# ZhengyiLuo/PHC

Measured on AMD Instinct MI355X. Metric: env-steps/sec at 4096 humanoid envs per GPU (VecEnv.step incl. resets), higher is better.
Workload: dtype f32

## Files before the change

### phc_amd/csrc/phc_im.h

```cpp
#pragma once
#include "phc_task.h"

namespace phc {

#if defined(PHC_SIM_PROFILE) && defined(__HIPCC__)
static __device__ unsigned long long g_phc_ptl[32];
static __device__ long long g_phc_ptl_env = -1;
#if defined(__HIP_DEVICE_COMPILE__)
#define PHC_PTL(i, ENV, LANE) if ((long long)(ENV) == g_phc_ptl_env) { __builtin_amdgcn_sched_barrier(0); __builtin_amdgcn_s_waitcnt(0); \
        const unsigned long long t_ = __builtin_readcyclecounter(); if ((LANE) == 0) g_phc_ptl[i] = t_; __builtin_amdgcn_sched_barrier(0); }
#else
#define PHC_PTL(i, ENV, LANE)
#endif
#else
#define PHC_PTL(i, ENV, LANE)
#endif

PHC_HD int64_t motion_id_of(const phc_im_buffers_t& buf, int64_t env) { return buf.sampled_motion_ids ? buf.sampled_motion_ids[env] : env; }

PHC_HD int phc_atomic_inc(int32_t* p) {
#if defined(__HIP_DEVICE_COMPILE__)
    return atomicAdd(p, 1);
#else
    int v;
#pragma omp atomic capture
    v = (*p)++;
    return v;
#endif
}

PHC_HD void amp_obs_from_frames_lane(const phc_motion_lib_t& lib, const phc_im_params_t& prm, int nb, int j, const FrameRef& fr, float* a);
PHC_HD void amp_obs_from_ref_lane(const phc_motion_lib_t& lib, const phc_im_params_t& prm, int nb, int j,
                                  int64_t mid, float t, float* a) {
    if (j < nb && prm.num_amp_obs_extra > 0 && prm.amp_obs_extra)
        obs_extra_lane(prm.amp_obs_extra + mid * prm.num_amp_obs_extra, prm.num_amp_obs_extra, j, nb, a + prm.num_amp_obs_per_step - prm.num_amp_obs_extra);
    amp_obs_from_frames_lane(lib, prm, nb, j, frame_ref(lib, mid, t), a);
}
PHC_HD void amp_obs_from_frames_lane(const phc_motion_lib_t& lib, const phc_im_params_t& prm, int nb, int j, const FrameRef& fr, float* a) {
    BodyState root = ref_body(lib, fr, 0);
    Q4 hinv = calc_heading_quat_inv(obs_root_rot(prm, root.rot));
    if (j == 0) amp_obs_root(prm, root.pos, root.rot, root.vel, root.angvel, hinv, a);
    if (j >= 1 && j < nb) {
        int slot = prm.amp_joint_slot[j];
        if (slot >= 0) {
            V3 dp, dv;
            if (prm.dofs_per_joint == 1) {
                ref_joint(lib, fr, j, &dp, &dv);
                amp_obs_joint(prm, slot, dp, dv, a);
            } else {
                Q4 lr;
                ref_joint_rot(lib, fr, j, &lr, &dv);
                amp_obs_joint_rot(prm, slot, lr, dv, a);
            }
        }
    }
    if (j < prm.num_key_bodies) {
        BodyState kb = ref_body(lib, fr, prm.key_body_ids[j]);
        amp_obs_key(prm, j, kb.pos, kb.vel, root.pos, hinv, a);
    }
}

PHC_HD void amp_obs_from_sim_lane(const phc_im_params_t& prm, const phc_sim_state_t& sim, int nb, int nd, int64_t env, int j,
                                  const BodyState& root, Q4 hinv, const int* dof_start_tab, float* a) {
    if (j < nb && prm.num_amp_obs_extra > 0 && prm.amp_obs_extra)
        obs_extra_lane(prm.amp_obs_extra + env * prm.num_amp_obs_extra, prm.num_amp_obs_extra, j, nb, a + prm.num_amp_obs_per_step - prm.num_amp_obs_extra);
    if (j == 0) amp_obs_root(prm, root.pos, root.rot, root.vel, root.angvel, hinv, a);
    if (j >= 1 && j < nb) {
        int slot = prm.amp_joint_slot[j];
        if (slot >= 0) {
            V3 dp, dv;
            ld_joint_state(sim, nd, env, dof_start_tab[j], prm.dofs_per_joint, &dp, &dv);
            amp_obs_joint(prm, slot, dp, dv, a);
        }
    }
    if (j < prm.num_key_bodies) {
        BodyState kb = load_body(sim.rigid_body_state, env, nb, prm.key_body_ids[j]);
        amp_obs_key(prm, j, kb.pos, kb.vel, root.pos, hinv, a);
    }
}

PHC_HD int64_t amp_env_stride(const phc_im_params_t& prm, const phc_im_buffers_t& buf) {
    return buf.amp_env_stride > 0 ? buf.amp_env_stride : (int64_t)prm.num_amp_obs_steps * prm.num_amp_obs_per_step;
}
PHC_HD void amp_shift_lane(const phc_im_params_t& prm, const phc_im_buffers_t& buf, int64_t env, int lane, int nl) {
    const int A = prm.num_amp_obs_per_step, S = prm.num_amp_obs_steps;
    if (buf.amp_obs_out + A == buf.amp_obs_in) return;
    const float* src = buf.amp_obs_in + env * amp_env_stride(prm, buf);
    float* dst = buf.amp_obs_out + env * amp_env_stride(prm, buf) + A;
    const int n = (S - 1) * A;
    if ((A & 3) == 0) {
        const float4* s4 = reinterpret_cast<const float4*>(src);
        float4* d4 = reinterpret_cast<float4*>(dst);
        int i = lane;
        for (; i + 3 * nl < n / 4; i += 4 * nl) {
            const float4 a = s4[i], b = s4[i + nl], c = s4[i + 2 * nl], e = s4[i + 3 * nl];
            d4[i] = a; d4[i + nl] = b; d4[i + 2 * nl] = c; d4[i + 3 * nl] = e;
        }
        for (; i < n / 4; i += nl) d4[i] = s4[i];
    } else {
        for (int i = lane; i < n; i += nl) dst[i] = src[i];
    }
}

struct ImStepCtx {
    int64_t progress;
    float t_rew; V3 goff_rew;
    float t0; V3 goff;
    float t1;
    float start, start_off;
    int pass_time;
    int cycled, cycle_cnt, recovery_cnt;
};

PHC_HD ImStepCtx im_post_prologue(const phc_motion_lib_t& lib, const phc_im_params_t& prm, const phc_sim_state_t& sim,
                                  const phc_im_buffers_t& buf, int64_t env, int64_t progress) {
    ImStepCtx c;
    const int64_t mid = motion_id_of(buf, env);
    c.start = buf.motion_start_times[env];
    c.start_off = buf.motion_start_times_offset[env];
    c.goff_rew = ld3(buf.global_offset + env * 3);
    c.goff = c.goff_rew;
    c.t_rew = motion_time(progress, prm.dt, c.start, c.start_off);
    c.t0 = c.t_rew;
    c.cycle_cnt = buf.cycle_counter ? (buf.cycle_counter[env] > 1 ? buf.cycle_counter[env] - 1 : 0) : 0;
    c.recovery_cnt = buf.recovery_counter ? (buf.recovery_counter[env] > 1 ? buf.recovery_counter[env] - 1 : 0) : 0;
    c.cycled = 0;
    const bool pass_len = c.t_rew >= lib.motion_lengths[mid];
    c.pass_time = pass_len ? 1 : 0;
    if (prm.cycle_motion) {
        c.pass_time = (progress >= (int64_t)prm.max_episode_length - 1) ? 1 : 0;
        if (pass_len) {
            c.cycled = 1;
            c.start_off = neg_progress_time(progress, prm.dt);
            c.start = sample_time_interval(lib, mid, buf.cycle_phase[env]);
            c.cycle_cnt = 60;
            const FrameRef fr = frame_ref(lib, mid, c.start);
            const V3 rp = ref_root_pos_lerp(lib, fr);
            const float* rs = sim.root_states + env * 13;
            c.goff.x = rs[0] - rp.x; c.goff.y = rs[1] - rp.y;
            if (buf.offset_rand && prm.cycle_motion_xp) {
                c.goff.x += buf.offset_rand[env * 2]; c.goff.y += buf.offset_rand[env * 2 + 1];
            } else if (buf.offset_rand && prm.zero_out_far && prm.zero_out_far_train) {
                float ox, oy;
                disk_offset(buf.offset_rand[env * 2], buf.offset_rand[env * 2 + 1], &ox, &oy);
                c.goff.x += ox; c.goff.y += oy;
            }
            c.t0 = motion_time(progress, prm.dt, c.start, c.start_off);
        }
    }
    c.progress = progress;
    if (c.recovery_cnt > 0) c.progress = progress - 1;
    c.t1 = motion_time(c.progress + 1, prm.dt, c.start, c.start_off);
    return c;
}

PHC_HD float zero_out_far_ref(const phc_im_params_t& prm, int slot, const BodyState& body, const BodyState& root,
                              const BodyState& ref_root, BodyState* ref) {
    const float distance = norm(root.pos - ref_root.pos);
    if (distance > prm.close_distance) {
        if (slot >= 1) { ref->pos = body.pos; ref->rot = body.rot; }
        ref->vel = body.vel; ref->angvel = body.angvel;
    }
    if (distance > prm.far_distance && slot == 0) {
        V3 d = ref->pos - body.pos;
        ref->pos = v3(d.x / distance * prm.far_distance, d.y / distance * prm.far_distance, d.z / distance * prm.far_distance) + body.pos;
    }
    return distance;
}

PHC_HD bool occluded(const phc_im_buffers_t& buf, const phc_im_params_t& prm, int64_t env, int slot) {
    return buf.occl_mask != nullptr && slot >= 0 && buf.occl_mask[env * prm.num_track_bodies + slot] != 0;
}
PHC_HD void occlude_ref(const phc_im_buffers_t& buf, const phc_im_params_t& prm, int64_t env, int slot, const BodyState& body, BodyState* rt) {
    if (!occluded(buf, prm, env, slot) || (prm.obs_v >= 1 && prm.obs_v <= 3)) return;
    if (prm.obs_v == 7) { rt->pos = body.pos; rt->rot = body.rot; }
    else *rt = body;
}

PHC_HD void task_obs_future_lane(const phc_motion_lib_t& lib, const phc_im_params_t& prm, int64_t mid, int64_t progress1, float start, float start_off,
                                 V3 goff, int slot, int j, const BodyState& body, const BodyState& root, float* tobs) {
    const int T = prm.num_traj_samples;
    if (T <= 1 || slot < 0 || !(prm.obs_v == 6 || prm.obs_v == 7 || prm.obs_v == 9)) return;
    const Q4 hroot = obs_root_rot(prm, root.rot);
    const Q4 hinv = calc_heading_quat_inv(hroot), h = calc_heading_quat(hroot);
    const int block = prm.num_task_obs / T;
    for (int k = 1; k < T; ++k) {
        PHC_NO_CONTRACT
        const float kts = (float)k * prm.traj_sample_timestep;
        BodyState r = ref_body(lib, frame_ref(lib, mid, motion_time_future(progress1, prm.dt, kts, start, start_off)), j);
        r.pos += goff;
        task_obs_lane(prm, slot, body, root, r, hinv, h, tobs + k * block);
    }
}

PHC_HD RewardPartial im_post_lane(const phc_model_t& model, const phc_motion_lib_t& lib, const phc_im_params_t& prm,
                                  const phc_sim_state_t& sim, const phc_im_buffers_t& buf, int64_t env, int j, const ImStepCtx& c,
                                  const FrameTab& tab, const BodyState& body, const BodyState& root) {
    const int nb = model.num_bodies, nd = model.num_dof;
    RewardPartial rp;
    rp.pos = rp.rot = rp.vel = rp.angvel = rp.power = rp.dist = rp.root_dist = 0.f; rp.fallen = 0;
    const int64_t mid = motion_id_of(buf, env);
    if (j >= nb) {
        const int e = j - nb;
        if (e >= prm.num_ext_bodies || prm.track_body_reward) return rp;
        const BodyState par = load_body(sim.rigid_body_state, env, nb, prm.ext_parent[e]);
        BodyState cur;
        cur.pos = quat_rotate(par.rot, ld3(prm.ext_offset + 3 * e)) + par.pos;
        cur.rot = par.rot;
        BodyState ref;
        ref_body_ext(lib, frame_ref(lib, mid, c.cycled ? c.t_rew : c.t0), e, &ref.pos, &ref.rot);
        ref.pos += c.cycled ? c.goff_rew : c.goff;
        const V3 d = ref.pos - cur.pos;
        rp.pos = (d.x * d.x + d.y * d.y + d.z * d.z) / 3.0f;
        const float ang = quat_to_angle_axis(quat_mul(ref.rot, quat_conjugate(cur.rot)), nullptr);
        rp.rot = ang * ang;
        return rp;
    }
    const FrameRef fr0 = frame_ref(tab, c.t0), fr1 = frame_ref(tab, c.t1);
    PHC_PTL(2, env, j)
    const BodyRaw q0 = ref_body_raw(lib, fr0, j), q1 = ref_body_raw(lib, fr1, j);
    JointPosRaw qj;
    const bool want_dof = buf.ref_dof_pos != nullptr && j >= 1;
    if (want_dof) qj = ref_joint_pos_raw(lib, fr1, j);
    PHC_PTL(3, env, j)
    const Q4 hroot = obs_root_rot(prm, root.rot);
    Q4 hinv = calc_heading_quat_inv(hroot), h = calc_heading_quat(hroot);
    float* obs = buf.obs_buf + env * (int64_t)(prm.num_self_obs + prm.num_task_obs);
    if (prm.self_obs_v == 2 && buf.body_state_hist) self_obs_v2_lane(prm, buf.body_state_hist, nb, env, j, body, root, hinv, obs, true, false);
    else self_obs_lane(prm, nb, j, body, root, hinv, obs, (sim.force_sensor && prm.self_obs_v == 3) ? sim.force_sensor + env * (int64_t)(prm.num_force_sensors * 6) : nullptr, env);
    PHC_PTL(4, env, j)
    {
        float* amp = buf.amp_obs_out + env * amp_env_stride(prm, buf);
        amp_obs_from_sim_lane(prm, sim, nb, nd, env, j, root, hinv, model.ints + 4 + 3 * PHC_MAX_BODIES, amp);
    }
    PHC_PTL(5, env, j)
    BodyState r0 = ref_body_blend(q0, fr0.blend), r1 = ref_body_blend(q1, fr1.blend);
    r0.pos += c.goff; r1.pos += c.goff;
    rp = reward_partial(prm, env, nb, j, body, r0);
    if (c.cycled) {
        BodyState rr = ref_body(lib, frame_ref(lib, mid, c.t_rew), j);
        rr.pos += c.goff_rew;
        RewardPartial q = reward_partial(prm, env, nb, j, body, rr);
        rp.pos = q.pos; rp.rot = q.rot; rp.vel = q.vel; rp.angvel = q.angvel;
        if (j == 0) rp.root_dist = norm(body.pos - rr.pos);
    } else if (j == 0) {
        rp.root_dist = norm(body.pos - r0.pos);
    }
    if (prm.track_body_reward && prm.track_slot[j] < 0) rp.pos = rp.rot = rp.vel = rp.angvel = 0.f;
    if (occluded(buf, prm, env, prm.track_slot[j])) { rp.dist = 0.f; rp.fallen = 0; }
    if (prm.power_reward && j >= 1) {
        int ds = model.ints[4 + 3 * PHC_MAX_BODIES + j];
        const float* d = sim.dof_state + (env * nd + ds) * 2;
        const float* f = sim.dof_force + env * nd + ds;
        rp.power = fabsf(f[0] * d[1]);
        if (prm.dofs_per_joint != 1) rp.power += fabsf(f[1] * d[3]) + fabsf(f[2] * d[5]);
    }
    PHC_PTL(6, env, j)
    int slot = prm.track_slot[j];
    if (slot >= 0) {
        BodyState rt = r1;
        if (prm.zero_out_far && !(prm.obs_v >= 1 && prm.obs_v <= 3)) {
            BodyState rroot = (j == 0) ? r1 : ref_body(lib, fr1, 0);
            if (j != 0) rroot.pos += c.goff;
            const float dist = zero_out_far_ref(prm, slot, body, root, rroot, &rt);
            if (j == 0 && buf.point_goal) buf.point_goal[env] = dist;
        }
        occlude_ref(buf, prm, env, slot, body, &rt);
        V3 jd = v3(0.f, 0.f, 0.f), jv, rjd = jd, rjv;
        if (prm.obs_v == 2 && j >= 1) {
            ld_joint_state(sim, nd, env, model.ints[4 + 3 * PHC_MAX_BODIES + j], prm.dofs_per_joint, &jd, &jv);
            ref_joint(lib, fr1, j, &rjd, &rjv);
        }
        task_obs_lane(prm, slot, body, root, rt, hinv, h, obs + prm.num_self_obs, &jd, &rjd);
    }
    PHC_PTL(7, env, j)
    if (buf.ref_body_pos) st3(buf.ref_body_pos + (env * nb + j) * 3, r1.pos);
    if (buf.ref_body_rot) st4(buf.ref_body_rot + (env * nb + j) * 4, r1.rot);
    if (buf.ref_body_vel) st3(buf.ref_body_vel + (env * nb + j) * 3, r1.vel);
    if (want_dof)
        st_joint(buf.ref_dof_pos + env * nd + model.ints[4 + 3 * PHC_MAX_BODIES + j], prm.dofs_per_joint, ref_joint_pos_blend(lib, qj, fr1.blend));
    PHC_PTL(8, env, j)
    if (prm.num_traj_samples > 1)
        task_obs_future_lane(lib, prm, mid, c.progress + 1, c.start, c.start_off, c.goff, prm.track_slot[j], j, load_body(sim.rigid_body_state, env, nb, j),
                             load_body(sim.rigid_body_state, env, nb, 0), buf.obs_buf + env * (int64_t)(prm.num_self_obs + prm.num_task_obs) + prm.num_self_obs);
    return rp;
}

PHC_HD void im_post_finalize(const phc_motion_lib_t& lib, const phc_im_params_t& prm, const phc_im_buffers_t& buf, int nb,
                             int64_t env, const ImStepCtx& c, int64_t progress, float s_pos, float s_rot, float s_vel, float s_angvel,
                             float s_power, float s_dist, float root_dist, float prev_point_goal, int any_fallen, int n_reset_bodies) {
    float J = (float)nb, JE = (float)(nb + prm.num_ext_bodies);
    if (prm.track_body_reward) J = JE = (float)prm.num_track_bodies;
    float r_pos = expf(-prm.k_pos * (s_pos / JE));
    float r_rot = expf(-prm.k_rot * (s_rot / JE));
    float r_vel = expf(-prm.k_vel * (s_vel / J));
    float r_ang = expf(-prm.k_ang_vel * (s_angvel / J));
    float rew = prm.w_pos * r_pos + prm.w_rot * r_rot + prm.w_vel * r_vel + prm.w_ang_vel * r_ang;
    const int nraw = prm.power_reward ? 5 : 4;
    float* raw = buf.reward_raw + env * nraw;
    if (prm.zero_out_far) {
        const float pg = fminf(prev_point_goal - root_dist, 1.0f / 3.0f) * 9.0f;
        const bool far = root_dist > 0.25f;
        raw[0] = pg + (far ? 0.f : r_pos * 0.5f);
        raw[1] = far ? 0.f : r_rot * 0.5f; raw[2] = far ? 0.f : r_vel * 0.5f; raw[3] = far ? 0.f : r_ang * 0.5f;
        rew = pg + (far ? 0.f : rew * 0.5f);
    } else {
        raw[0] = r_pos; raw[1] = r_rot; raw[2] = r_vel; raw[3] = r_ang;
    }
    if (prm.power_reward) {
        float pr = -prm.power_coefficient * s_power;
        if (progress <= 3) pr = 0.f;
        rew += pr;
        raw[4] = pr;
    }
    buf.rew_buf[env] = rew;
    int fallen = any_fallen;
    if (prm.use_mean_termination) {
        float mean = s_dist / (float)n_reset_bodies;
        fallen = mean > prm.termination_distances[prm.first_reset_body] ? 1 : 0;
    }
    int64_t terminated = 0;
    if (prm.enable_early_termination) {
        if (!(progress > 1)) fallen = 0;
        if (prm.disable_collision_check) fallen = 0;
        terminated = fallen ? 1 : 0;
    }
    int64_t reset = c.pass_time ? 1 : terminated;
    if (!c.pass_time && c.cycle_cnt > 0) { reset = 0; terminated = 0; }
    if (c.recovery_cnt > 0) { reset = 0; terminated = 0; }
    buf.terminate_buf[env] = terminated;
    buf.reset_buf[env] = reset;
    if (reset && buf.reset_list) {
        const int sub = (int)((env >> 3) & (PHC_RESET_SUBLISTS - 1));
        const int i = phc_atomic_inc(buf.reset_count + (buf.reset_slot * PHC_RESET_SUBLISTS + sub) * PHC_RESET_COUNT_STRIDE);
        buf.reset_list[sub * buf.reset_sublist_cap + i] = (int32_t)env;
    }
    buf.progress_buf[env] = c.progress;
    if (buf.cycle_counter) buf.cycle_counter[env] = c.cycle_cnt;
    if (buf.recovery_counter) buf.recovery_counter[env] = c.recovery_cnt;
    if (c.cycled) {
        buf.motion_start_times[env] = c.start;
        buf.motion_start_times_offset[env] = c.start_off;
        st3(buf.global_offset + env * 3, c.goff);
    }
}

PHC_HD void im_reset_lane(const phc_model_t& model, const phc_motion_lib_t& lib, const phc_im_params_t& prm,
                          const phc_sim_state_t& sim, const phc_im_buffers_t& buf, int64_t env, int j, float t, bool clear_reset_flag,
                          int parts = 3) {
    const int nb = model.num_bodies, nd = model.num_dof;
    const int64_t mid = motion_id_of(buf, env);
    const bool p_state = (parts & 1) != 0, p_task = (parts & 2) != 0;
    if (j < nb) {
        const FrameRef fr = frame_ref(lib, mid, t);
        BodyState rs = ref_body(lib, fr, j);
        BodyState root = (j == 0) ? rs : ref_body(lib, fr, 0);
        if (p_state) {
        store_body(sim.rigid_body_state, env, nb, j, rs);
        if (sim.contact_force) st3(sim.contact_force + (env * nb + j) * 3, v3(0.f, 0.f, 0.f));
        if (j == 0) {
            float* r = sim.root_states + env * 13;
            st3(r, rs.pos); st4(r + 3, rs.rot); st3(r + 7, rs.vel); st3(r + 10, rs.angvel);
        } else {
            V3 dp, dv;
            ref_joint(lib, fr, j, &dp, &dv);
            const int ds = model.ints[4 + 3 * PHC_MAX_BODIES + j];
            float* d = sim.dof_state + (env * nd + ds) * 2;
            d[0] = dp.x; d[1] = dv.x;
            if (prm.dofs_per_joint != 1) { d[2] = dp.y; d[3] = dv.y; d[4] = dp.z; d[5] = dv.z; }
            st_joint(sim.pd_target + env * nd + ds, prm.dofs_per_joint, dp);
            if (sim.dof_force) st_joint(sim.dof_force + env * nd + ds, prm.dofs_per_joint, v3(0.f, 0.f, 0.f));
        }
        }
        const Q4 hroot = obs_root_rot(prm, root.rot);
        Q4 hinv = calc_heading_quat_inv(hroot), h = calc_heading_quat(hroot);
        float* obs = buf.obs_buf + env * (int64_t)(prm.num_self_obs + prm.num_task_obs);
        if (p_state) {
        if (prm.self_obs_v == 2 && buf.body_state_hist) self_obs_v2_lane(prm, buf.body_state_hist, nb, env, j, rs, root, hinv, obs, false, true);
        else self_obs_lane(prm, nb, j, rs, root, hinv, obs, (sim.force_sensor && prm.self_obs_v == 3) ? sim.force_sensor + env * (int64_t)(prm.num_force_sensors * 6) : nullptr, env);
        }
        if (p_task) {
        const float t1 = motion_time(1, prm.dt, t, 0.f);
        const FrameRef fr1 = frame_ref(lib, mid, t1);
        BodyState r1 = ref_body(lib, fr1, j);
        V3 goff = v3(0.f, 0.f, 0.f);
        if (buf.offset_rand && prm.zero_out_far && prm.zero_out_far_train)
            disk_offset(buf.offset_rand[env * 2], buf.offset_rand[env * 2 + 1], &goff.x, &goff.y);
        r1.pos += goff;
        int slot = prm.track_slot[j];
        if (slot >= 0) {
            BodyState rt = r1;
            if (prm.zero_out_far && !(prm.obs_v >= 1 && prm.obs_v <= 3)) {
                BodyState rroot = (j == 0) ? r1 : ref_body(lib, fr1, 0);
                if (j != 0) rroot.pos += goff;
                const float dist = zero_out_far_ref(prm, slot, rs, root, rroot, &rt);
                if (j == 0 && buf.point_goal) buf.point_goal[env] = dist;
            }
            occlude_ref(buf, prm, env, slot, rs, &rt);
            V3 jd = v3(0.f, 0.f, 0.f), jv, rjd = jd, rjv;
            if (prm.obs_v == 2 && j >= 1) { ref_joint(lib, fr, j, &jd, &jv); ref_joint(lib, fr1, j, &rjd, &rjv); }
            task_obs_lane(prm, slot, rs, root, rt, hinv, h, obs + prm.num_self_obs, &jd, &rjd);
        }
        if (buf.ref_body_pos) st3(buf.ref_body_pos + (env * nb + j) * 3, r1.pos);
        if (buf.ref_body_rot) st4(buf.ref_body_rot + (env * nb + j) * 4, r1.rot);
        if (buf.ref_body_vel) st3(buf.ref_body_vel + (env * nb + j) * 3, r1.vel);
        if (buf.ref_dof_pos && j >= 1) {
            V3 dp, dv;
            ref_joint(lib, fr1, j, &dp, &dv);
            st_joint(buf.ref_dof_pos + env * nd + model.ints[4 + 3 * PHC_MAX_BODIES + j], prm.dofs_per_joint, dp);
        }
        if (prm.num_traj_samples > 1) {
            const FrameRef frt = frame_ref(lib, mid, t);
            V3 go = v3(0.f, 0.f, 0.f);
            if (buf.offset_rand && prm.zero_out_far && prm.zero_out_far_train) disk_offset(buf.offset_rand[env * 2], buf.offset_rand[env * 2 + 1], &go.x, &go.y);
            task_obs_future_lane(lib, prm, mid, 1, t, 0.f, go, prm.track_slot[j], j, ref_body(lib, frt, j), ref_body(lib, frt, 0),
                                 buf.obs_buf + env * (int64_t)(prm.num_self_obs + prm.num_task_obs) + prm.num_self_obs);
        }
        }
    }
    if (j == 0 && p_state) {
        buf.motion_start_times[env] = t;
        buf.motion_start_times_offset[env] = 0.f;
        V3 goff = v3(0.f, 0.f, 0.f);
        const bool far_start = buf.offset_rand && prm.zero_out_far && prm.zero_out_far_train;
        if (far_start) disk_offset(buf.offset_rand[env * 2], buf.offset_rand[env * 2 + 1], &goff.x, &goff.y);
        st3(buf.global_offset + env * 3, goff);
        buf.progress_buf[env] = 0; buf.terminate_buf[env] = 0;
        if (clear_reset_flag) buf.reset_buf[env] = 0;
        if (buf.cycle_counter) buf.cycle_counter[env] = far_start ? prm.zero_out_far_steps : 0;
        if (buf.recovery_counter) buf.recovery_counter[env] = 0;
    }
}

PHC_HD void im_reset_from_state_lane(const phc_model_t& model, const phc_motion_lib_t& lib, const phc_im_params_t& prm,
                                     const phc_sim_state_t& sim, const phc_im_buffers_t& buf, int64_t env, int j, int fill_history) {
    const int nb = model.num_bodies, nd = model.num_dof;
    const int64_t mid = motion_id_of(buf, env);
    const int S = prm.num_amp_obs_steps, A = prm.num_amp_obs_per_step;
    if (j < nb) {
        BodyState body = load_body(sim.rigid_body_state, env, nb, j);
        BodyState root = load_body(sim.rigid_body_state, env, nb, 0);
        if (sim.contact_force) st3(sim.contact_force + (env * nb + j) * 3, v3(0.f, 0.f, 0.f));
        if (j >= 1) {
            const int ds = model.ints[4 + 3 * PHC_MAX_BODIES + j];
            V3 dp, dv;
            ld_joint_state(sim, nd, env, ds, prm.dofs_per_joint, &dp, &dv);
            st_joint(sim.pd_target + env * nd + ds, prm.dofs_per_joint, dp);
        }
        const V3 goff = ld3(buf.global_offset + env * 3);
        const float t1 = motion_time(1, prm.dt, buf.motion_start_times[env], buf.motion_start_times_offset[env]);
        const FrameRef fr1 = frame_ref(lib, mid, t1);
        BodyState r1 = ref_body(lib, fr1, j);
        r1.pos += goff;
        const Q4 hroot = obs_root_rot(prm, root.rot);
    Q4 hinv = calc_heading_quat_inv(hroot), h = calc_heading_quat(hroot);
        float* obs = buf.obs_buf + env * (int64_t)(prm.num_self_obs + prm.num_task_obs);
        if (prm.self_obs_v == 2 && buf.body_state_hist) self_obs_v2_lane(prm, buf.body_state_hist, nb, env, j, body, root, hinv, obs, false, true);
        else self_obs_lane(prm, nb, j, body, root, hinv, obs, (sim.force_sensor && prm.self_obs_v == 3) ? sim.force_sensor + env * (int64_t)(prm.num_force_sensors * 6) : nullptr, env);
        int slot = prm.track_slot[j];
        if (slot >= 0) {
            BodyState rt = r1;
            if (prm.zero_out_far && !(prm.obs_v >= 1 && prm.obs_v <= 3)) {
                BodyState rroot = (j == 0) ? r1 : ref_body(lib, fr1, 0);
                if (j != 0) rroot.pos += goff;
                const float dist = zero_out_far_ref(prm, slot, body, root, rroot, &rt);
                if (j == 0 && buf.point_goal) buf.point_goal[env] = dist;
            }
            occlude_ref(buf, prm, env, slot, body, &rt);
            V3 jd = v3(0.f, 0.f, 0.f), jv, rjd = jd, rjv;
            if (prm.obs_v == 2 && j >= 1) {
                ld_joint_state(sim, nd, env, model.ints[4 + 3 * PHC_MAX_BODIES + j], prm.dofs_per_joint, &jd, &jv);
                ref_joint(lib, fr1, j, &rjd, &rjv);
            }
            task_obs_lane(prm, slot, body, root, rt, hinv, h, obs + prm.num_self_obs, &jd, &rjd);
        }
        if (buf.ref_body_pos) st3(buf.ref_body_pos + (env * nb + j) * 3, r1.pos);
        if (buf.ref_body_rot) st4(buf.ref_body_rot + (env * nb + j) * 4, r1.rot);
        if (buf.ref_body_vel) st3(buf.ref_body_vel + (env * nb + j) * 3, r1.vel);
        if (buf.ref_dof_pos && j >= 1) {
            V3 dp, dv;
            ref_joint(lib, fr1, j, &dp, &dv);
            st_joint(buf.ref_dof_pos + env * nd + model.ints[4 + 3 * PHC_MAX_BODIES + j], prm.dofs_per_joint, dp);
        }
        float* amp = buf.amp_obs_out + env * amp_env_stride(prm, buf);
        const int nfill = fill_history ? S : 1;
        for (int k = 0; k < nfill; ++k)
            amp_obs_from_sim_lane(prm, sim, nb, nd, env, j, root, hinv, model.ints + 4 + 3 * PHC_MAX_BODIES, amp + k * A);
        if (prm.num_traj_samples > 1)
            task_obs_future_lane(lib, prm, mid, 1, buf.motion_start_times[env], buf.motion_start_times_offset[env], ld3(buf.global_offset + env * 3),
                                 prm.track_slot[j], j, load_body(sim.rigid_body_state, env, nb, j), load_body(sim.rigid_body_state, env, nb, 0),
                                 buf.obs_buf + env * (int64_t)(prm.num_self_obs + prm.num_task_obs) + prm.num_self_obs);
    }
    if (j == 0) {
        buf.progress_buf[env] = 0; buf.terminate_buf[env] = 0; buf.reset_buf[env] = 0;
    }
}

PHC_HD void im_reset_amp_lane(const phc_motion_lib_t& lib, const phc_im_params_t& prm, const phc_im_buffers_t& buf, int nb,
                              int64_t env, int j, float t, int k) {
    const int A = prm.num_amp_obs_per_step;
    float* amp = buf.amp_obs_out + env * amp_env_stride(prm, buf);
    amp_obs_from_ref_lane(lib, prm, nb, j, motion_id_of(buf, env), history_time(t, prm.dt, k), amp + k * A);
}
#define PHC_AMP_TABLE_BLEND_TOL 1e-4f
PHC_HD void amp_obs_from_table_lane(const phc_motion_lib_t& lib, const phc_im_params_t& prm, int nb, int j, int nl, int64_t mid, float t, float* a) {
    const int A = prm.num_amp_obs_per_step, E = prm.num_amp_obs_extra, W = A - E;
    const FrameRef fr = frame_ref(lib, mid, t);
    const float b = fr.blend;
    if (j < nb && E > 0 && prm.amp_obs_extra) obs_extra_lane(prm.amp_obs_extra + mid * E, E, j, nb, a + W);
    if (!(b <= PHC_AMP_TABLE_BLEND_TOL)) {
        amp_obs_from_frames_lane(lib, prm, nb, j, fr, a);
        return;
    }
    const float* r0 = prm.amp_ref_table + fr.f0 * (int64_t)W;
    const float* r1 = prm.amp_ref_table + fr.f1 * (int64_t)W;
    const float s0 = 1.0f - b;
    for (int c0 = j; c0 < W; c0 += 8 * nl) {
        float u[8], v[8];
        for (int i = 0; i < 8; ++i) { const int c = c0 + i * nl; if (c < W) { u[i] = r0[c]; v[i] = r1[c]; } }
        for (int i = 0; i < 8; ++i) { const int c = c0 + i * nl; if (c < W) a[c] = s0 * u[i] + b * v[i]; }
    }
}
PHC_HD void im_reset_amp_table_lane(const phc_motion_lib_t& lib, const phc_im_params_t& prm, const phc_im_buffers_t& buf, int nb,
                                    int64_t env, int j, int nl, float t, int k) {
    amp_obs_from_table_lane(lib, prm, nb, j, nl, motion_id_of(buf, env), history_time(t, prm.dt, k),
                            buf.amp_obs_out + env * amp_env_stride(prm, buf) + k * prm.num_amp_obs_per_step);
}

}
```

### phc_amd/csrc/phc_kernels.hip

```cpp
#include <hip/hip_runtime.h>
#include <stdlib.h>
#include "phc_aba.h"
#include "phc_im.h"
#include "phc_group.h"

using namespace phc;

template <int DPJ>
__device__ __forceinline__ void pin_family(phc_motion_lib_t& lib, phc_im_params_t& prm) {
    lib.dofs_per_joint = DPJ; prm.dofs_per_joint = DPJ;
    if (DPJ == 3) { lib.num_ext_bodies = 0; prm.num_ext_bodies = 0; }
}

template <int DPJ, int G>
__global__ __launch_bounds__(256) void k_im_post_physics(phc_model_t model, phc_motion_lib_t lib, phc_im_params_t prm,
                                                        phc_sim_state_t sim, phc_im_buffers_t buf, int n_reset_bodies) {
    pin_family<DPJ>(lib, prm);
    const int lane = threadIdx.x & (G - 1);
    const int64_t env = ((int64_t)blockIdx.x * blockDim.x + threadIdx.x) / G;
    if (env >= sim.num_envs) return;
    PHC_PTL(0, env, lane)
    if (blockIdx.x == 0 && threadIdx.x == 0 && buf.reset_rng_counter) *buf.reset_rng_counter += 1;
    const int64_t progress = buf.progress_buf[env] + 1;
    const FrameTab tab = frame_tab(lib, motion_id_of(buf, env));
    const int jb = lane < model.num_bodies ? lane : 0;
    const BodyState body = load_body(sim.rigid_body_state, env, model.num_bodies, jb);
    const BodyState root = load_body(sim.rigid_body_state, env, model.num_bodies, 0);
    const ImStepCtx c = im_post_prologue(lib, prm, sim, buf, env, progress);
    const float prev_goal = (prm.zero_out_far && buf.point_goal) ? buf.point_goal[env] : 0.f;
    PHC_PTL(1, env, lane)
    RewardPartial rp = im_post_lane(model, lib, prm, sim, buf, env, lane, c, tab, body, root);
    PHC_PTL(9, env, lane)
    amp_shift_lane(prm, buf, env, lane, G);
    float s_pos = group_sum<G>(rp.pos), s_rot = group_sum<G>(rp.rot), s_vel = group_sum<G>(rp.vel), s_ang = group_sum<G>(rp.angvel);
    float s_pow = group_sum<G>(rp.power), s_dist = group_sum<G>(rp.dist);
    int fallen = group_or<G>(rp.fallen);
    PHC_PTL(10, env, lane)
    if (lane == 0)
        im_post_finalize(lib, prm, buf, model.num_bodies, env, c, progress, s_pos, s_rot, s_vel, s_ang, s_pow, s_dist, rp.root_dist,
                         prev_goal, fallen, n_reset_bodies);
    PHC_PTL(11, env, lane)
}
#ifdef PHC_SIM_PROFILE
extern "C" int32_t phc_debug_post_timeline(unsigned long long* out32, long long env) {
    if (out32 && hipMemcpyFromSymbol(out32, HIP_SYMBOL(phc::g_phc_ptl), sizeof(unsigned long long) * 32) != hipSuccess) return -1;
    unsigned long long z[32] = {0};
    if (hipMemcpyToSymbol(HIP_SYMBOL(phc::g_phc_ptl), z, sizeof(z)) != hipSuccess) return -1;
    return hipMemcpyToSymbol(HIP_SYMBOL(phc::g_phc_ptl_env), &env, sizeof(env)) == hipSuccess ? 0 : -1;
}
#endif

template <int DPJ, int G>
__global__ __launch_bounds__(256) void k_amp_ref_table(phc_model_t model, phc_motion_lib_t lib, phc_im_params_t prm, int64_t num_frames,
                                                       const int64_t* __restrict__ next_frame, float* __restrict__ table) {
    pin_family<DPJ>(lib, prm);
    const int lane = threadIdx.x & (G - 1);
    const int64_t f = ((int64_t)blockIdx.x * blockDim.x + threadIdx.x) / G;
    if (f >= num_frames) return;
    FrameRef fr;
    fr.f0 = f; fr.f1 = next_frame[f]; fr.idx0 = fr.idx1 = 0; fr.blend = 0.f;
    amp_obs_from_frames_lane(lib, prm, model.num_bodies, lane, fr, table + f * (int64_t)(prm.num_amp_obs_per_step - prm.num_amp_obs_extra));
}

template <int G>
__global__ __launch_bounds__(256) void k_im_reset_from_state(phc_model_t model, phc_motion_lib_t lib, phc_im_params_t prm, phc_sim_state_t sim,
                                                            phc_im_buffers_t buf, int num_reset, const int64_t* __restrict__ env_ids,
                                                            int fill_history) {
    const int lane = threadIdx.x & (G - 1);
    const int64_t r = ((int64_t)blockIdx.x * blockDim.x + threadIdx.x) / G;
    if (r >= num_reset) return;
    im_reset_from_state_lane(model, lib, prm, sim, buf, env_ids[r], lane, fill_history);
}

__device__ __forceinline__ float hash_u01(uint64_t key, uint32_t env) {
    uint32_t x = env * 0x9E3779B1u ^ (uint32_t)key;
    x ^= x >> 16; x *= 0x85EBCA6Bu; x ^= x >> 13; x *= 0xC2B2AE35u; x ^= x >> 16;
    x += (uint32_t)(key >> 32);
    x ^= x >> 15; x *= 0x2C1B3C6Du; x ^= x >> 12; x *= 0x297A2D39u; x ^= x >> 15;
    return (float)(x >> 8) * (1.0f / 16777216.0f);
}
__host__ __device__ static inline uint64_t splitmix64(uint64_t z) {
    z += 0x9E3779B97F4A7C15ull;
    z = (z ^ (z >> 30)) * 0xBF58476D1CE4E5B9ull;
    z = (z ^ (z >> 27)) * 0x94D049BB133111EBull;
    return z ^ (z >> 31);
}

#ifdef PHC_SIM_PROFILE
__device__ unsigned long long g_phc_rtl[64];
__device__ int g_phc_rtl_group = -1;
extern "C" int32_t phc_debug_reset_timeline(unsigned long long* out64, int32_t group) {
    if (out64 && hipMemcpyFromSymbol(out64, HIP_SYMBOL(g_phc_rtl), sizeof(g_phc_rtl)) != hipSuccess) return -1;
    unsigned long long z[64] = {0};
    if (hipMemcpyToSymbol(HIP_SYMBOL(g_phc_rtl), z, sizeof(z)) != hipSuccess) return -1;
    return hipMemcpyToSymbol(HIP_SYMBOL(g_phc_rtl_group), &group, sizeof(group)) == hipSuccess ? 0 : -1;
}
#define PHC_RTL(i) if (rtl_on) { __builtin_amdgcn_sched_barrier(0); __builtin_amdgcn_s_waitcnt(0); const unsigned long long t_ = __builtin_readcyclecounter(); \
        if (lane == 0) g_phc_rtl[i] = t_; __builtin_amdgcn_sched_barrier(0); }
#else
#define PHC_RTL(i)
#endif

template <int DPJ, bool RNG, int G>
__global__ __launch_bounds__(256) void k_im_reset(phc_model_t model, phc_motion_lib_t lib, phc_im_params_t prm, phc_sim_state_t sim,
                                                 phc_im_buffers_t buf, int num_reset, const int64_t* __restrict__ env_ids,
                                                 const float* __restrict__ phase, int start_at_zero, uint64_t rng_key) {
    pin_family<DPJ>(lib, prm);
    const int lane = threadIdx.x & (G - 1);
    const int64_t r = ((int64_t)blockIdx.x * blockDim.x + threadIdx.x) / G;
    const int k = (int)blockIdx.y;
#ifdef PHC_SIM_PROFILE
    const bool rtl_on = (int)(r * 16 + k) == g_phc_rtl_group;
#endif
    PHC_RTL(0)
    int64_t env;
    if (RNG && buf.reset_list) {
        const int cap = buf.reset_sublist_cap, r32 = (int)r;
        const int sub = r32 & (PHC_RESET_SUBLISTS - 1), i = r32 >> 4;
        if (r32 < PHC_RESET_SUBLISTS && k == 0 && lane == 0)
            buf.reset_count[(((buf.reset_slot + 1) % 3) * PHC_RESET_SUBLISTS + r32) * PHC_RESET_COUNT_STRIDE] = 0;
        if (i >= cap || i >= buf.reset_count[(buf.reset_slot * PHC_RESET_SUBLISTS + sub) * PHC_RESET_COUNT_STRIDE]) return;
        env = buf.reset_list[sub * cap + i];
    } else {
        if (r >= num_reset) return;
        env = env_ids ? env_ids[r] : r;
        if (!env_ids && buf.reset_buf[env] == 0) return;
    }
    PHC_RTL(1)
    const int64_t mid = motion_id_of(buf, env);
    const uint64_t key = (RNG && buf.reset_rng_counter) ? splitmix64(rng_key ^ (*buf.reset_rng_counter * 0x9E6C63D0876A9A47ull)) : rng_key;
    const float t = start_at_zero ? 0.f : sample_time_interval(lib, mid, RNG ? hash_u01(key, (uint32_t)env) : phase[r]);
    PHC_RTL(2)
    if (k < 2) im_reset_lane(model, lib, prm, sim, buf, env, lane, t, env_ids != nullptr, 1 << k);
    PHC_RTL(3)
    if (k >= 2) {
        if (prm.amp_ref_table != nullptr) im_reset_amp_table_lane(lib, prm, buf, model.num_bodies, env, lane, G, t, k - 2);
        else im_reset_amp_lane(lib, prm, buf, model.num_bodies, env, lane, t, k - 2);
    }
    PHC_RTL(4)
}

template <int G>
__global__ __launch_bounds__(256) void k_amp_obs_demo(phc_model_t model, phc_motion_lib_t lib, phc_im_params_t prm, int n,
                                                     const int64_t* __restrict__ motion_ids, const float* __restrict__ times0,
                                                     float* __restrict__ out) {
    const int lane = threadIdx.x & (G - 1);
    const int64_t i = ((int64_t)blockIdx.x * blockDim.x + threadIdx.x) / G;
    const int k = (int)blockIdx.y;
    const int S = prm.num_amp_obs_steps, A = prm.num_amp_obs_per_step;
    if (i >= n) return;
    if (prm.amp_ref_table != nullptr) amp_obs_from_table_lane(lib, prm, model.num_bodies, lane, G, motion_ids[i], history_time(times0[i], prm.dt, k), out + (i * S + k) * A);
    else amp_obs_from_ref_lane(lib, prm, model.num_bodies, lane, motion_ids[i], history_time(times0[i], prm.dt, k), out + (i * S + k) * A);
}

template <int G>
__global__ __launch_bounds__(256) void k_motion_state(phc_motion_lib_t lib, int n, const int64_t* __restrict__ ids,
                                                     const float* __restrict__ times, const float* __restrict__ offset,
                                                     float* rg_pos, float* rb_rot, float* body_vel, float* body_ang_vel,
                                                     float* dof_pos, float* dof_vel, int64_t* idx0, int64_t* idx1, float* blend,
                                                     float* rg_pos_ext, float* rb_rot_ext) {
    const int lane = threadIdx.x & (G - 1);
    const int64_t i = ((int64_t)blockIdx.x * blockDim.x + threadIdx.x) / G;
    if (i >= n) return;
    const int nb = lib.num_bodies;
    const FrameRef fr = frame_ref(lib, ids[i], times[i]);
    if (lane == 0) {
        if (idx0) idx0[i] = fr.idx0;
        if (idx1) idx1[i] = fr.idx1;
        if (blend) blend[i] = fr.blend;
    }
    if (lane >= nb) {
        const int e = lane - nb, ne = lib.num_ext_bodies;
        if (e < ne && (rg_pos_ext || rb_rot_ext)) {
            V3 p; Q4 q;
            ref_body_ext(lib, fr, e, &p, &q);
            if (offset) p += ld3(offset + i * 3);
            if (rg_pos_ext) st3(rg_pos_ext + (i * ne + e) * 3, p);
            if (rb_rot_ext) st4(rb_rot_ext + (i * ne + e) * 4, q);
        }
        return;
    }
    BodyState s = ref_body(lib, fr, lane);
    if (offset) s.pos += ld3(offset + i * 3);
    if (rg_pos) st3(rg_pos + (i * nb + lane) * 3, s.pos);
    if (rb_rot) st4(rb_rot + (i * nb + lane) * 4, s.rot);
    if (body_vel) st3(body_vel + (i * nb + lane) * 3, s.vel);
    if (body_ang_vel) st3(body_ang_vel + (i * nb + lane) * 3, s.angvel);
    if (lane >= 1 && (dof_pos || dof_vel)) {
        V3 dp, dv;
        ref_joint(lib, fr, lane, &dp, &dv);
        const int dpj = lib.dofs_per_joint == 1 ? 1 : 3;
        if (dof_pos) st_joint(dof_pos + (i * (nb - 1) + (lane - 1)) * dpj, dpj, dp);
        if (dof_vel) st_joint(dof_vel + (i * (nb - 1) + (lane - 1)) * dpj, dpj, dv);
    }
}

__global__ void k_sample_time_interval(phc_motion_lib_t lib, int n, const int64_t* __restrict__ ids,
                                       const float* __restrict__ phase, float* __restrict__ out) {
    const int i = blockIdx.x * blockDim.x + threadIdx.x;
    if (i < n) out[i] = sample_time_interval(lib, ids[i], phase[i]);
}

__global__ void k_gae(int T, int n, const float* __restrict__ fdones, const float* __restrict__ values,
                      const float* __restrict__ rewards, const float* __restrict__ next_values, float gamma, float tau,
                      float* __restrict__ advs) {
    const int i = blockIdx.x * blockDim.x + threadIdx.x;
    if (i >= n) return;
    float last = 0.f;
    for (int t = T - 1; t >= 0; --t) {
        const int64_t k = (int64_t)t * n + i;
        const float not_done = 1.0f - fdones[k];
        const float delta = rewards[k] + gamma * next_values[k] - values[k];
        last = delta + gamma * tau * not_done * last;
        advs[k] = last;
    }
}

__device__ __forceinline__ Q4 pl_quat_mul_norm(Q4 a, Q4 b) {
    Q4 q = quat_mul16(a, b);
    if (q.w < 0.f) q = q4(-q.x, -q.y, -q.z, -q.w);
    float n = fmaxf(sqrtf(q.x * q.x + q.y * q.y + q.z * q.z + q.w * q.w), 1e-9f);
    return q4(q.x / n, q.y / n, q.z / n, q.w / n);
}
__global__ void k_fk(phc_model_t model, int64_t T, const float* __restrict__ local_rot, const float* __restrict__ root_trans,
                     float* __restrict__ grot, float* __restrict__ gpos) {
    const int64_t f = (int64_t)blockIdx.x * blockDim.x + threadIdx.x;
    if (f >= T) return;
    const int nb = model.num_bodies;
    for (int j = 0; j < nb; ++j) {
        const int p = model_tab(model, 0, j);
        Q4 lq = ld4(local_rot + (f * nb + j) * 4);
        if (p < 0) {
            st4(grot + (f * nb + j) * 4, lq);
            st3(gpos + (f * nb + j) * 3, ld3(root_trans + f * 3));
        } else {
            Q4 pq = ld4(grot + (f * nb + p) * 4);
            const float* mb = model_body(model, j);
            V3 off = quat_rotate(pq, v3(mb[0], mb[1], mb[2]));
            st4(grot + (f * nb + j) * 4, pl_quat_mul_norm(pq, lq));
            st3(gpos + (f * nb + j) * 3, off + ld3(gpos + (f * nb + p) * 3));
        }
    }
}

static inline int32_t launch_status() {
    hipError_t e = hipGetLastError();
    return e == hipSuccess ? 0 : (int32_t)e;
}
static inline int env_blocks(int64_t groups, int lanes) { return (int)((groups * lanes + 255) / 256); }
static inline int group_lanes(int num_bodies, int num_ext) { return num_bodies + num_ext > 32 ? 64 : 32; }

extern "C" {

int32_t phc_abi_version(void) { return PHC_ABI_VERSION; }

int32_t phc_motion_state(const phc_motion_lib_t* lib, int32_t n, const int64_t* motion_ids, const float* motion_times,
                         const float* offset, float* rg_pos, float* rb_rot, float* body_vel, float* body_ang_vel,
                         float* dof_pos, float* dof_vel, int64_t* frame_idx0, int64_t* frame_idx1, float* blend, float* rg_pos_ext,
                         float* rb_rot_ext, void* stream) {
    if (!lib || n < 0 || lib->num_bodies + lib->num_ext_bodies > PHC_MAX_BODIES) return PHC_EINVAL;
    if (n == 0) return 0;
    if (group_lanes(lib->num_bodies, lib->num_ext_bodies) == 64)
        hipLaunchKernelGGL(k_motion_state<64>, dim3(env_blocks(n, 64)), dim3(256), 0, (hipStream_t)stream, *lib, n, motion_ids, motion_times, offset,
                           rg_pos, rb_rot, body_vel, body_ang_vel, dof_pos, dof_vel, frame_idx0, frame_idx1, blend, rg_pos_ext, rb_rot_ext);
    else
        hipLaunchKernelGGL(k_motion_state<32>, dim3(env_blocks(n, 32)), dim3(256), 0, (hipStream_t)stream, *lib, n, motion_ids, motion_times, offset,
                           rg_pos, rb_rot, body_vel, body_ang_vel, dof_pos, dof_vel, frame_idx0, frame_idx1, blend, rg_pos_ext, rb_rot_ext);
    return launch_status();
}

int32_t phc_sample_time_interval(const phc_motion_lib_t* lib, int32_t n, const int64_t* motion_ids, const float* phase,
                                 float* motion_times, void* stream) {
    if (!lib || n < 0) return PHC_EINVAL;
    if (n == 0) return 0;
    hipLaunchKernelGGL(k_sample_time_interval, dim3((n + 255) / 256), dim3(256), 0, (hipStream_t)stream, *lib, n, motion_ids, phase, motion_times);
    return launch_status();
}

static int32_t check_model(const phc_model_t* m) {
    if (!m || m->num_bodies < 1 || m->num_bodies > PHC_MAX_BODIES || !m->ints || !m->floats) return PHC_EINVAL;
    if (m->num_dof != 3 * (m->num_bodies - 1) && m->num_dof != m->num_bodies - 1) return PHC_EUNSUPPORTED;
    return 0;
}

static int32_t check_im(const phc_model_t* model, const phc_motion_lib_t* lib, const phc_im_params_t* prm) {
    int32_t rc = check_model(model);
    if (rc) return rc;
    if (!lib || !prm || lib->num_bodies != model->num_bodies) return PHC_EINVAL;
    const int dpj = model->num_dof == model->num_bodies - 1 && model->num_bodies > 2 ? 1 : 3;
    if ((lib->dofs_per_joint == 1 ? 1 : 3) != dpj || (prm->dofs_per_joint == 1 ? 1 : 3) != dpj) return PHC_EINVAL;
    if (prm->num_ext_bodies < 0 || prm->num_ext_bodies != lib->num_ext_bodies || model->num_bodies + prm->num_ext_bodies > PHC_MAX_BODIES) return PHC_EINVAL;
    if (prm->num_ext_bodies > 0 && (!prm->ext_parent || !prm->ext_offset)) return PHC_EINVAL;
    if (!prm->track_slot || !prm->reset_mask || !prm->termination_distances || !prm->key_body_ids || !prm->amp_joint_slot) return PHC_EINVAL;
    if (prm->num_key_bodies > 32) return PHC_EUNSUPPORTED;
    return 0;
}

int32_t phc_im_post_physics(const phc_model_t* model, const phc_motion_lib_t* lib, const phc_im_params_t* prm,
                            const phc_sim_state_t* sim, const phc_im_buffers_t* buf, void* stream) {
    int32_t rc = check_im(model, lib, prm);
    if (rc) return rc;
    if (!sim || !buf || buf->amp_obs_in == buf->amp_obs_out) return PHC_EINVAL;
    if (prm->cycle_motion && (!buf->cycle_counter || !buf->cycle_phase)) return PHC_EINVAL;
    if (prm->zero_out_far && (!buf->point_goal || prm->track_slot == nullptr)) return PHC_EINVAL;
    if (sim->num_envs == 0) return 0;
    const int n_reset_bodies = prm->num_reset_bodies > 0 ? prm->num_reset_bodies : 1;
    const int g = group_lanes(model->num_bodies, prm->num_ext_bodies);
    const dim3 grid(env_blocks(sim->num_envs, g));
#define PHC_POST(DPJ, G) hipLaunchKernelGGL((k_im_post_physics<DPJ, G>), grid, dim3(256), 0, (hipStream_t)stream, *model, *lib, *prm, *sim, *buf, n_reset_bodies)
    if (prm->dofs_per_joint == 1) { if (g == 64) PHC_POST(1, 64); else PHC_POST(1, 32); }
    else { if (g == 64) PHC_POST(3, 64); else PHC_POST(3, 32); }
#undef PHC_POST
    return launch_status();
}

int32_t phc_amp_ref_table(const phc_model_t* model, const phc_motion_lib_t* lib, const phc_im_params_t* prm, int64_t num_frames,
                          const int64_t* next_frame, float* table, void* stream) {
    int32_t rc = check_im(model, lib, prm);
    if (rc) return rc;
    if (!table || !next_frame || num_frames < 0 || num_frames > lib->num_frames_total) return PHC_EINVAL;
    if (num_frames == 0) return 0;
    const int g = group_lanes(model->num_bodies, prm->num_ext_bodies);
    const int64_t blocks = (num_frames * g + 255) / 256;
    if (blocks > 0x7fffffffLL) return PHC_EUNSUPPORTED;
#define PHC_TAB(DPJ, G) hipLaunchKernelGGL((k_amp_ref_table<DPJ, G>), dim3((unsigned)blocks), dim3(256), 0, (hipStream_t)stream, *model, *lib, *prm, num_frames, next_frame, table)
    if (prm->dofs_per_joint == 1) { if (g == 64) PHC_TAB(1, 64); else PHC_TAB(1, 32); }
    else { if (g == 64) PHC_TAB(3, 64); else PHC_TAB(3, 32); }
#undef PHC_TAB
    return launch_status();
}

int32_t phc_im_reset(const phc_model_t* model, const phc_motion_lib_t* lib, const phc_im_params_t* prm, const phc_sim_state_t* sim,
                     const phc_im_buffers_t* buf, int32_t num_reset, const int64_t* env_ids, const float* phase,
                     int32_t start_at_zero, void* stream) {
    int32_t rc = check_im(model, lib, prm);
    if (rc) return rc;
    if (!sim || !buf || num_reset < 0 || (!start_at_zero && !phase)) return PHC_EINVAL;
    if (num_reset == 0) return 0;
    const int g = group_lanes(model->num_bodies, prm->num_ext_bodies);
    const dim3 grid(env_blocks(num_reset, g), prm->num_amp_obs_steps + 2);
#define PHC_RESET(DPJ, G) hipLaunchKernelGGL((k_im_reset<DPJ, false, G>), grid, dim3(256), 0, (hipStream_t)stream, *model, *lib, *prm, *sim, *buf, num_reset, env_ids, phase, start_at_zero, 0ull)
    if (prm->dofs_per_joint == 1) { if (g == 64) PHC_RESET(1, 64); else PHC_RESET(1, 32); }
    else { if (g == 64) PHC_RESET(3, 64); else PHC_RESET(3, 32); }
#undef PHC_RESET
    return launch_status();
}

int32_t phc_im_reset_done(const phc_model_t* model, const phc_motion_lib_t* lib, const phc_im_params_t* prm, const phc_sim_state_t* sim,
                          const phc_im_buffers_t* buf, uint64_t seed, uint64_t counter, int32_t start_at_zero, void* stream) {
    int32_t rc = check_im(model, lib, prm);
    if (rc) return rc;
    if (!sim || !buf) return PHC_EINVAL;
    if (sim->num_envs == 0) return 0;
    if (buf->reset_list && (!buf->reset_count || buf->reset_sublist_cap * PHC_RESET_SUBLISTS < sim->num_envs)) return PHC_EINVAL;
    const int n = buf->reset_list ? buf->reset_sublist_cap * PHC_RESET_SUBLISTS : sim->num_envs;
    const uint64_t key = splitmix64(splitmix64(seed) ^ ((buf->reset_rng_counter ? 0ull : counter) * 0xD1342543DE82EF95ull));
    const int g = group_lanes(model->num_bodies, prm->num_ext_bodies);
    const dim3 grid(env_blocks(n, g), prm->num_amp_obs_steps + 2);
#define PHC_RESET(DPJ, G) hipLaunchKernelGGL((k_im_reset<DPJ, true, G>), grid, dim3(256), 0, (hipStream_t)stream, *model, *lib, *prm, *sim, *buf, n, nullptr, nullptr, start_at_zero, key)
    if (prm->dofs_per_joint == 1) { if (g == 64) PHC_RESET(1, 64); else PHC_RESET(1, 32); }
    else { if (g == 64) PHC_RESET(3, 64); else PHC_RESET(3, 32); }
#undef PHC_RESET
    return launch_status();
}

int32_t phc_im_reset_from_state(const phc_model_t* model, const phc_motion_lib_t* lib, const phc_im_params_t* prm,
                                const phc_sim_state_t* sim, const phc_im_buffers_t* buf, int32_t num_reset, const int64_t* env_ids,
                                int32_t fill_history, void* stream) {
    int32_t rc = check_im(model, lib, prm);
    if (rc) return rc;
    if (!sim || !buf || num_reset < 0 || (num_reset > 0 && !env_ids)) return PHC_EINVAL;
    if (num_reset == 0) return 0;
    if (group_lanes(model->num_bodies, prm->num_ext_bodies) == 64)
        hipLaunchKernelGGL(k_im_reset_from_state<64>, dim3(env_blocks(num_reset, 64)), dim3(256), 0, (hipStream_t)stream, *model, *lib, *prm, *sim,
                           *buf, num_reset, env_ids, fill_history);
    else
        hipLaunchKernelGGL(k_im_reset_from_state<32>, dim3(env_blocks(num_reset, 32)), dim3(256), 0, (hipStream_t)stream, *model, *lib, *prm, *sim,
                           *buf, num_reset, env_ids, fill_history);
    return launch_status();
}

int32_t phc_amp_obs_demo(const phc_model_t* model, const phc_motion_lib_t* lib, const phc_im_params_t* prm, int32_t n,
                         const int64_t* motion_ids, const float* motion_times0, float* amp_obs_demo, void* stream) {
    int32_t rc = check_im(model, lib, prm);
    if (rc) return rc;
    if (n < 0) return PHC_EINVAL;
    if (n == 0) return 0;
    if (group_lanes(model->num_bodies, prm->num_ext_bodies) == 64)
        hipLaunchKernelGGL(k_amp_obs_demo<64>, dim3(env_blocks(n, 64), prm->num_amp_obs_steps), dim3(256), 0, (hipStream_t)stream, *model, *lib,
                           *prm, n, motion_ids, motion_times0, amp_obs_demo);
    else
        hipLaunchKernelGGL(k_amp_obs_demo<32>, dim3(env_blocks(n, 32), prm->num_amp_obs_steps), dim3(256), 0, (hipStream_t)stream, *model, *lib,
                           *prm, n, motion_ids, motion_times0, amp_obs_demo);
    return launch_status();
}

int32_t phc_gae(int32_t horizon, int32_t n, const float* fdones, const float* values, const float* rewards,
                const float* next_values, float gamma, float tau, float* advs, void* stream) {
    if (horizon < 0 || n < 0) return PHC_EINVAL;
    if (horizon == 0 || n == 0) return 0;
    hipLaunchKernelGGL(k_gae, dim3((n + 255) / 256), dim3(256), 0, (hipStream_t)stream, horizon, n, fdones, values, rewards,
                       next_values, gamma, tau, advs);
    return launch_status();
}

int32_t phc_fk(const phc_model_t* model, int64_t num_frames, const float* local_rot, const float* root_trans, float* global_rot,
               float* global_pos, void* stream) {
    if (!model || model->num_bodies < 1 || model->num_bodies > PHC_MAX_BODIES || num_frames < 0) return PHC_EINVAL;
    if (num_frames == 0) return 0;
    hipLaunchKernelGGL(k_fk, dim3((unsigned)((num_frames + 255) / 256)), dim3(256), 0, (hipStream_t)stream, *model, num_frames,
                       local_rot, root_trans, global_rot, global_pos);
    return launch_status();
}

}
```

Measured before the change: 38.05 million.

## Merge AMP history rows into one reset role and flatten reset grid

When an AMP reference table exists, the reset kernel now uses three roles per env instead of one per AMP history step plus two. The single AMP role loops over all history steps and prefetches the next step's table rows while writing the current one. The 2D grid becomes 1D, with the role interleaved with the env block index so the roles of the same env sit in adjacent blocks. This cuts block count and per-block setup (env lookup, RNG, time sampling). In exchange the per-thread AMP work becomes serial across steps, which may lengthen the critical path.

```diff
diff --git a/phc_amd/csrc/phc_im.h b/phc_amd/csrc/phc_im.h
--- a/phc_amd/csrc/phc_im.h
+++ b/phc_amd/csrc/phc_im.h
@@ -526,5 +526,50 @@
     amp_obs_from_table_lane(lib, prm, nb, j, nl, motion_id_of(buf, env), history_time(t, prm.dt, k),
                             buf.amp_obs_out + env * amp_env_stride(prm, buf) + k * prm.num_amp_obs_per_step);
 }
-
-}
+PHC_HD void im_reset_amp_table_rows_lane(const phc_motion_lib_t& lib, const phc_im_params_t& prm, const phc_im_buffers_t& buf, int nb,
+                                         int64_t env, int j, int nl, float t) {
+    const int S = prm.num_amp_obs_steps, A = prm.num_amp_obs_per_step, E = prm.num_amp_obs_extra, W = A - E;
+    const int64_t mid = motion_id_of(buf, env);
+    const FrameTab tab = frame_tab(lib, mid);
+    float* amp = buf.amp_obs_out + env * amp_env_stride(prm, buf);
+    float u[8], v[8], nu[8], nv[8];
+    bool have = false;
+    FrameRef fr = frame_ref(tab, history_time(t, prm.dt, 0));
+    for (int k = 0; k < S; ++k) {
+        float* a = amp + k * A;
+        const float b = fr.blend;
+        FrameRef nx = fr;
+        if (k + 1 < S) nx = frame_ref(tab, history_time(t, prm.dt, k + 1));
+        bool nhave = false;
+        if (b <= PHC_AMP_TABLE_BLEND_TOL) {
+            const float* r0 = prm.amp_ref_table + fr.f0 * (int64_t)W;
+            const float* r1 = prm.amp_ref_table + fr.f1 * (int64_t)W;
+            if (!have)
+                for (int i = 0; i < 8; ++i) { const int c = j + i * nl; if (c < W) { u[i] = r0[c]; v[i] = r1[c]; } }
+            if (k + 1 < S && nx.blend <= PHC_AMP_TABLE_BLEND_TOL) {
+                const float* n0 = prm.amp_ref_table + nx.f0 * (int64_t)W;
+                const float* n1 = prm.amp_ref_table + nx.f1 * (int64_t)W;
+                for (int i = 0; i < 8; ++i) { const int c = j + i * nl; if (c < W) { nu[i] = n0[c]; nv[i] = n1[c]; } }
+                nhave = true;
+            }
+            if (j < nb && E > 0 && prm.amp_obs_extra) obs_extra_lane(prm.amp_obs_extra + mid * E, E, j, nb, a + W);
+            const float s0 = 1.0f - b;
+            for (int i = 0; i < 8; ++i) { const int c = j + i * nl; if (c < W) a[c] = s0 * u[i] + b * v[i]; }
+            for (int c0 = j + 8 * nl; c0 < W; c0 += 8 * nl) {
+                float p[8], q[8];
+                for (int i = 0; i < 8; ++i) { const int c = c0 + i * nl; if (c < W) { p[i] = r0[c]; q[i] = r1[c]; } }
+                for (int i = 0; i < 8; ++i) { const int c = c0 + i * nl; if (c < W) a[c] = s0 * p[i] + b * q[i]; }
+            }
+        } else {
+            if (j < nb && E > 0 && prm.amp_obs_extra) obs_extra_lane(prm.amp_obs_extra + mid * E, E, j, nb, a + W);
+            amp_obs_from_frames_lane(lib, prm, nb, j, fr, a);
+            for (int i = 0; i < 8; ++i) u[i] = v[i] = 0.f;
+        }
+        fr = nx;
+        have = nhave;
+        if (nhave)
+            for (int i = 0; i < 8; ++i) { u[i] = nu[i]; v[i] = nv[i]; }
+    }
+}
+
+}
diff --git a/phc_amd/csrc/phc_kernels.hip b/phc_amd/csrc/phc_kernels.hip
--- a/phc_amd/csrc/phc_kernels.hip
+++ b/phc_amd/csrc/phc_kernels.hip
@@ -104,11 +104,11 @@
 template <int DPJ, bool RNG, int G>
 __global__ __launch_bounds__(256) void k_im_reset(phc_model_t model, phc_motion_lib_t lib, phc_im_params_t prm, phc_sim_state_t sim,
                                                  phc_im_buffers_t buf, int num_reset, const int64_t* __restrict__ env_ids,
-                                                 const float* __restrict__ phase, int start_at_zero, uint64_t rng_key) {
+                                                 const float* __restrict__ phase, int start_at_zero, uint64_t rng_key, int roles) {
     pin_family<DPJ>(lib, prm);
     const int lane = threadIdx.x & (G - 1);
-    const int64_t r = ((int64_t)blockIdx.x * blockDim.x + threadIdx.x) / G;
-    const int k = (int)blockIdx.y;
+    const int xb = (int)(blockIdx.x / (unsigned)roles), k = (int)(blockIdx.x % (unsigned)roles);
+    const int64_t r = ((int64_t)xb * blockDim.x + threadIdx.x) / G;
 #ifdef PHC_SIM_PROFILE
     const bool rtl_on = (int)(r * 16 + k) == g_phc_rtl_group;
 #endif
@@ -134,7 +134,7 @@
     if (k < 2) im_reset_lane(model, lib, prm, sim, buf, env, lane, t, env_ids != nullptr, 1 << k);
     PHC_RTL(3)
     if (k >= 2) {
-        if (prm.amp_ref_table != nullptr) im_reset_amp_table_lane(lib, prm, buf, model.num_bodies, env, lane, G, t, k - 2);
+        if (prm.amp_ref_table != nullptr) im_reset_amp_table_rows_lane(lib, prm, buf, model.num_bodies, env, lane, G, t);
         else im_reset_amp_lane(lib, prm, buf, model.num_bodies, env, lane, t, k - 2);
     }
     PHC_RTL(4)
@@ -249,6 +249,7 @@
 }
 static inline int env_blocks(int64_t groups, int lanes) { return (int)((groups * lanes + 255) / 256); }
 static inline int group_lanes(int num_bodies, int num_ext) { return num_bodies + num_ext > 32 ? 64 : 32; }
+static inline int reset_roles(const phc_im_params_t* prm) { return prm->amp_ref_table ? 3 : prm->num_amp_obs_steps + 2; }
 
 extern "C" {
 
@@ -338,8 +339,9 @@
     if (!sim || !buf || num_reset < 0 || (!start_at_zero && !phase)) return PHC_EINVAL;
     if (num_reset == 0) return 0;
     const int g = group_lanes(model->num_bodies, prm->num_ext_bodies);
-    const dim3 grid(env_blocks(num_reset, g), prm->num_amp_obs_steps + 2);
-#define PHC_RESET(DPJ, G) hipLaunchKernelGGL((k_im_reset<DPJ, false, G>), grid, dim3(256), 0, (hipStream_t)stream, *model, *lib, *prm, *sim, *buf, num_reset, env_ids, phase, start_at_zero, 0ull)
+    const int roles = reset_roles(prm);
+    const dim3 grid(env_blocks(num_reset, g) * roles);
+#define PHC_RESET(DPJ, G) hipLaunchKernelGGL((k_im_reset<DPJ, false, G>), grid, dim3(256), 0, (hipStream_t)stream, *model, *lib, *prm, *sim, *buf, num_reset, env_ids, phase, start_at_zero, 0ull, roles)
     if (prm->dofs_per_joint == 1) { if (g == 64) PHC_RESET(1, 64); else PHC_RESET(1, 32); }
     else { if (g == 64) PHC_RESET(3, 64); else PHC_RESET(3, 32); }
 #undef PHC_RESET
@@ -356,8 +358,9 @@
     const int n = buf->reset_list ? buf->reset_sublist_cap * PHC_RESET_SUBLISTS : sim->num_envs;
     const uint64_t key = splitmix64(splitmix64(seed) ^ ((buf->reset_rng_counter ? 0ull : counter) * 0xD1342543DE82EF95ull));
     const int g = group_lanes(model->num_bodies, prm->num_ext_bodies);
-    const dim3 grid(env_blocks(n, g), prm->num_amp_obs_steps + 2);
-#define PHC_RESET(DPJ, G) hipLaunchKernelGGL((k_im_reset<DPJ, true, G>), grid, dim3(256), 0, (hipStream_t)stream, *model, *lib, *prm, *sim, *buf, n, nullptr, nullptr, start_at_zero, key)
+    const int roles = reset_roles(prm);
+    const dim3 grid(env_blocks(n, g) * roles);
+#define PHC_RESET(DPJ, G) hipLaunchKernelGGL((k_im_reset<DPJ, true, G>), grid, dim3(256), 0, (hipStream_t)stream, *model, *lib, *prm, *sim, *buf, n, nullptr, nullptr, start_at_zero, key, roles)
     if (prm->dofs_per_joint == 1) { if (g == 64) PHC_RESET(1, 64); else PHC_RESET(1, 32); }
     else { if (g == 64) PHC_RESET(3, 64); else PHC_RESET(3, 32); }
 #undef PHC_RESET
```

Result: slower. 35.27 million (-7.3%).
